# thnak/image_super_resolution

Measured on AMD Instinct MI355X. Metric: 4x SR megapixels/sec (HR output) + PSNR vs reference CPU path, higher is better.
Workload: dtype fp16; 1 GPU; ResNet(16, 0.2, scaleRate=4) RRDB inference, 128x128->512x512; global_batch=16, per_gpu_batch=16, lr_size=128, scale=4, parallelism=dp1 (independent tile shards), streams_per_gpu=1, hip_graph=True, trunk=persistent chain kernel, storage=fp16 activations and packed weights, fp32 accumulation

## Files before the change

### image_super_resolution_amd/csrc/capi.hip

```cpp
#include <stdarg.h>
#include <stdio.h>
#include <string.h>

#include "isr_common.h"

namespace isr {
int conv3x3_fwd_dispatch(const isr_conv_desc* d, hipStream_t s);
int conv3x3_fwd_variant(const isr_conv_desc* d, int variant, hipStream_t s);
int conv_stamps_set(void* p);
size_t trunk_state_words(int n, int ha, int wa);
int trunk_launch(const isr_chain_desc* c, hipStream_t s);
int trunk_stamps_set(void* p);
int trunk_knobs_set(const int* k);
int trunk_item_stamps_set(void* p);
size_t conv3x3_packed_bytes(int cout, int cin);
int conv3x3_pack(const float* w, void* out, int cout, int cin, hipStream_t s);
int conv3x3_pack_f16(const float* w, void* out, int cout, int cin, hipStream_t s);
size_t conv3x3_wino_packed_bytes(int cout, int cin);
int conv3x3_wino_pack(const float* w, void* out, int cout, int cin, hipStream_t s);
int conv3x3_wino_fwd_dispatch(const isr_conv_desc* d, hipStream_t s);
int head9x9_fwd_dispatch(const isr_head_desc* d, hipStream_t s);
int tail9x9_fwd_dispatch(const isr_tail_desc* d, hipStream_t s);
int tail9x9_fwd_variant(const isr_tail_desc* d, int variant, hipStream_t s);
size_t head9x9_packed_bytes(int cout);
// ... 32 lines not shown

static thread_local char g_err[512] = "";

static int fail(int code, const char* fmt, ...) __attribute__((format(printf, 2, 3)));
static int fail(int code, const char* fmt, ...) {
    va_list ap;
    va_start(ap, fmt);
    vsnprintf(g_err, sizeof(g_err), fmt, ap);
    va_end(ap);
    return code;
}

static int launched(int rc, const char* what) {
    if (rc != 0) {
        hipError_t e = hipGetLastError();
        return fail(ISR_ERR_LAUNCH, "%s: launch failed: %s", what, hipGetErrorString(e));
    }
    g_err[0] = 0;
    return ISR_OK;
}

static bool view_ok(const isr_view& v, int ha, int wa, int halo, int ch, const char* name, int align16) {
    if (!v.data) { fail(ISR_ERR_BAD_DESC, "%s: null data", name); return false; }
    if (v.pad < halo) { fail(ISR_ERR_BAD_DESC, "%s: pad %d < required halo %d", name, v.pad, halo); return false; }
    if (v.hp < ha + 2 * v.pad || v.wp < wa + 2 * v.pad) {
        fail(ISR_ERR_BAD_DESC, "%s: buffer %dx%d (pad %d) smaller than computed region %dx%d", name, v.hp, v.wp, v.pad, ha, wa);
        return false;
    }
    if (v.coff < 0 || v.coff + ch > v.cs) {
        fail(ISR_ERR_BAD_DESC, "%s: channels [%d,%d) exceed stride %d", name, v.coff, v.coff + ch, v.cs);
        return false;
    }
    if (align16 && ((v.cs % 16) || (v.coff % 16) || ((uintptr_t)v.data % 16))) {
        fail(ISR_ERR_BAD_DESC, "%s: channel count/offset must be multiples of 16 (channel-blocked layout) "
             "and data 16-byte aligned", name);
        return false;
    }
    return true;
}

extern "C" {

const char* isr_last_error(void) { return g_err; }

int isr_pack_conv3x3_batch(const isr_pack_item* items, int32_t n, isr_stream_t s) {
    if (!items || n <= 0 || n > 65535) return fail(ISR_ERR_BAD_DESC, "pack_conv3x3_batch: bad item table (n=%d)", n);
    return launched(isr::conv3x3_pack_batch(items, n, (hipStream_t)s), "pack_conv3x3_batch");
}

static int mt_ok(const isr_mt_tensor* ts, const isr_mt_chunk* cs, int32_t n, const char* what) {
    if (!ts || !cs) return fail(ISR_ERR_BAD_DESC, "%s: null tensor / chunk table", what);
    if (n <= 0 || n > (1 << 30)) return fail(ISR_ERR_BAD_DESC, "%s: bad chunk count %d", what, n);
    return ISR_OK;
}

int isr_mt_adam_guarded(const isr_mt_tensor* ts, const isr_mt_chunk* cs, int32_t n, const isr_adam_args* a,
                        const float* scale, const uint32_t* guard, isr_stream_t s) {
    if (int rc = mt_ok(ts, cs, n, "mt_adam")) return rc;
    if (!a) return fail(ISR_ERR_BAD_DESC, "mt_adam: null args");
    if (!(a->bc2_sqrt > 0.f) || !(a->beta1 >= 0.f && a->beta1 < 1.f) || !(a->beta2 >= 0.f && a->beta2 < 1.f))
        return fail(ISR_ERR_BAD_DESC, "mt_adam: bad betas / bias correction");
    return launched(isr::mt_adam_dispatch(ts, cs, n, a, scale, guard, (hipStream_t)s), "mt_adam");
}

int isr_mt_adam(const isr_mt_tensor* ts, const isr_mt_chunk* cs, int32_t n, const isr_adam_args* a,
                const float* scale, isr_stream_t s) {
    return isr_mt_adam_guarded(ts, cs, n, a, scale, nullptr, s);
}

int isr_mt_sumsq(const isr_mt_tensor* ts, const isr_mt_chunk* cs, int32_t n, float* partial, isr_stream_t s) {
    if (int rc = mt_ok(ts, cs, n, "mt_sumsq")) return rc;
    if (!partial) return fail(ISR_ERR_BAD_DESC, "mt_sumsq: null partial buffer");
    return launched(isr::mt_sumsq_dispatch(ts, cs, n, partial, (hipStream_t)s), "mt_sumsq");
}

int isr_clip_coef(const float* partial, int32_t n, float max_norm, float* out, isr_stream_t s) {
    if (!partial || !out || n <= 0) return fail(ISR_ERR_BAD_DESC, "clip_coef: bad arguments");
    return launched(isr::clip_coef_dispatch(partial, n, max_norm, out, (hipStream_t)s), "clip_coef");
}

int isr_mt_scale(const isr_mt_tensor* ts, const isr_mt_chunk* cs, int32_t n, const float* coef, isr_stream_t s) {
    if (int rc = mt_ok(ts, cs, n, "mt_scale")) return rc;
    if (!coef) return fail(ISR_ERR_BAD_DESC, "mt_scale: null coefficient");
    return launched(isr::mt_axpby_dispatch(ts, cs, n, 0, coef, 0.f, nullptr, (hipStream_t)s), "mt_scale");
}

int isr_mt_lerp_guarded(const isr_mt_tensor* ts, const isr_mt_chunk* cs, int32_t n, float d, const uint32_t* guard,
                        isr_stream_t s) {
    if (int rc = mt_ok(ts, cs, n, "mt_lerp")) return rc;
    return launched(isr::mt_axpby_dispatch(ts, cs, n, 1, nullptr, d, guard, (hipStream_t)s), "mt_lerp");
}

int isr_mt_lerp(const isr_mt_tensor* ts, const isr_mt_chunk* cs, int32_t n, float d, isr_stream_t s) {
    return isr_mt_lerp_guarded(ts, cs, n, d, nullptr, s);
}
int isr_version(void) { return 1; }

size_t isr_conv3x3_packed_bytes(int32_t cout, int32_t cin) { return isr::conv3x3_packed_bytes(cout, cin); }
size_t isr_head9x9_packed_bytes(int32_t cout, int32_t cin) { (void)cin; return isr::head9x9_packed_bytes(cout); }
size_t isr_tail9x9_packed_bytes(int32_t cout, int32_t cin) { (void)cout; (void)cin; return isr::tail9x9_packed_bytes(); }

int isr_pack_conv3x3(const float* w, void* packed, int32_t cout, int32_t cin, isr_stream_t s) {
    if (!w || !packed) return fail(ISR_ERR_BAD_DESC, "pack_conv3x3: null pointer");
    if (cin <= 0 || cin % 16) return fail(ISR_ERR_UNSUPPORTED, "pack_conv3x3: cin %d must be a positive multiple of 16", cin);
    if (cout <= 0 || cout % 32)
        return fail(ISR_ERR_UNSUPPORTED, "pack_conv3x3: cout %d must be a positive multiple of 32", cout);
    return launched(isr::conv3x3_pack(w, packed, cout, cin, (hipStream_t)s), "pack_conv3x3");
}

int isr_pack_conv3x3_dgrad(const float* w, void* packed, int32_t cout, int32_t cin, float scale, int32_t sub2,
                           isr_stream_t s) {
    if (!w || !packed) return fail(ISR_ERR_BAD_DESC, "pack_conv3x3_dgrad: null pointer");
    if (cin <= 0 || cin % 32 || cout <= 0 || cout % 32)
        return fail(ISR_ERR_UNSUPPORTED, "pack_conv3x3_dgrad: cin %d / cout %d must be multiples of 32", cin, cout);
    if (sub2 && cout % 128) return fail(ISR_ERR_UNSUPPORTED, "pack_conv3x3_dgrad: sub2 needs cout %% 128 == 0");
    return launched(isr::conv3x3_pack_dgrad(w, packed, cout, cin, scale, sub2, (hipStream_t)s), "pack_conv3x3_dgrad");
}

static int pack_head_any(const float* w, void* packed, int32_t cout, int32_t cin, isr_stream_t s, bool h) {
    if (!w || !packed) return fail(ISR_ERR_BAD_DESC, "pack_head9x9: null pointer");
    if (cout != 64 || cin < 1 || cin > 3) return fail(ISR_ERR_UNSUPPORTED, "pack_head9x9: need cout 64, cin <= 3 (got %d, %d)", cout, cin);
    return launched(isr::head9x9_pack(w, packed, cout, cin, (hipStream_t)s, h), "pack_head9x9");
}
int isr_pack_head9x9(const float* w, void* packed, int32_t cout, int32_t cin, isr_stream_t s) {
    return pack_head_any(w, packed, cout, cin, s, false);
}
int isr_pack_head9x9_f16(const float* w, void* packed, int32_t cout, int32_t cin, isr_stream_t s) {
    return pack_head_any(w, packed, cout, cin, s, true);
}

static int pack_tail_any(const float* w, void* packed, int32_t cout, int32_t cin, isr_stream_t s, bool h) {
    if (!w || !packed) return fail(ISR_ERR_BAD_DESC, "pack_tail9x9: null pointer");
    if (cout != 3 || cin != 64) return fail(ISR_ERR_UNSUPPORTED, "pack_tail9x9: need cout 3, cin 64 (got %d, %d)", cout, cin);
    return launched(isr::tail9x9_pack(w, packed, cout, cin, (hipStream_t)s, h), "pack_tail9x9");
}
int isr_pack_tail9x9(const float* w, void* packed, int32_t cout, int32_t cin, isr_stream_t s) {
    return pack_tail_any(w, packed, cout, cin, s, false);
}
int isr_pack_tail9x9_f16(const float* w, void* packed, int32_t cout, int32_t cin, isr_stream_t s) {
    return pack_tail_any(w, packed, cout, cin, s, true);
}

int isr_pack_conv3x3_f16(const float* w, void* packed, int32_t cout, int32_t cin, isr_stream_t s) {
    if (!w || !packed) return fail(ISR_ERR_BAD_DESC, "pack_conv3x3_f16: null pointer");
    if (cin <= 0 || cin % 16) return fail(ISR_ERR_UNSUPPORTED, "pack_conv3x3_f16: cin %d must be a positive multiple of 16", cin);
    if (cout <= 0 || cout % 32)
        return fail(ISR_ERR_UNSUPPORTED, "pack_conv3x3_f16: cout %d must be a positive multiple of 32", cout);
    return launched(isr::conv3x3_pack_f16(w, packed, cout, cin, (hipStream_t)s), "pack_conv3x3_f16");
}

static int conv3x3_validate(const isr_conv_desc* d) {
    if (!d) return fail(ISR_ERR_BAD_DESC, "conv3x3: null descriptor");
    if (d->n <= 0 || d->h <= 0 || d->w <= 0) return fail(ISR_ERR_BAD_DESC, "conv3x3: empty problem n=%d h=%d w=%d", d->n, d->h, d->w);
    if (d->ha % ISR_TILE_H || d->wa % ISR_TILE_W || d->ha < d->h || d->wa < d->w)
        return fail(ISR_ERR_BAD_DESC, "conv3x3: computed region %dx%d must cover %dx%d and be a multiple of %dx%d", d->ha, d->wa,
                    d->h, d->w, ISR_TILE_H, ISR_TILE_W);
    if (d->cin <= 0 || d->cin % 16) return fail(ISR_ERR_UNSUPPORTED, "conv3x3: cin %d must be a multiple of 16", d->cin);
    if (d->cout <= 0 || d->cout % 32)
        return fail(ISR_ERR_UNSUPPORTED, "conv3x3: cout %d must be a positive multiple of 32", d->cout);
    if (!d->wpack) return fail(ISR_ERR_BAD_DESC, "conv3x3: null weights");
    if (d->shuffle != 1 && d->shuffle != 2) return fail(ISR_ERR_UNSUPPORTED, "conv3x3: shuffle must be 1 or 2");
    if (d->taps < 0 || d->taps > 2) return fail(ISR_ERR_UNSUPPORTED, "conv3x3: taps must be 0, 1 or 2");
    if (d->taps && d->cout % 64) return fail(ISR_ERR_UNSUPPORTED, "conv3x3: a 2x2 tap window needs cout %% 64 == 0");
    if (d->x_sub2) {
        if (d->cin % 128) return fail(ISR_ERR_UNSUPPORTED, "conv3x3: x_sub2 needs cin %% 128 == 0 (got %d)", d->cin);
        if (d->shuffle != 1) return fail(ISR_ERR_UNSUPPORTED, "conv3x3: x_sub2 with a shuffled store");
        if (!view_ok(d->x, 2 * d->ha, 2 * d->wa, 2, d->cin / 4, "conv3x3.x", 1)) return ISR_ERR_BAD_DESC;
    } else if (!view_ok(d->x, d->ha, d->wa, 1, d->cin, "conv3x3.x", 1)) {
        return ISR_ERR_BAD_DESC;
    }
    if (d->m.data) {
        if (d->y2.data) return fail(ISR_ERR_UNSUPPORTED, "conv3x3: mask epilogue takes no second output");
        if (d->m_c0 < 0 || d->m_c0 % 32) return fail(ISR_ERR_BAD_DESC, "conv3x3: m_c0 %d must be a multiple of 32", d->m_c0);
        if (d->shuffle == 2) {
            if (d->m_c0) return fail(ISR_ERR_UNSUPPORTED, "conv3x3: a shuffled store masks all channels (m_c0 = 0)");
            if (!view_ok(d->m, 2 * d->ha, 2 * d->wa, 0, d->cout / 4, "conv3x3.m", 1)) return ISR_ERR_BAD_DESC;
        } else if (!view_ok(d->m, d->ha, d->wa, 0, d->cout, "conv3x3.m", 1)) {
            return ISR_ERR_BAD_DESC;
        }
    }
    if (d->r1_cn < 0 || d->r1_cn % 32) return fail(ISR_ERR_BAD_DESC, "conv3x3: r1_cn %d must be a multiple of 32", d->r1_cn);
    if (d->shuffle == 2) {
        if (d->cout % 64) return fail(ISR_ERR_UNSUPPORTED, "conv3x3: pixel shuffle needs cout %% 64 == 0");
        if (d->r1.data || d->r2.data || d->y2.data)
            return fail(ISR_ERR_UNSUPPORTED, "conv3x3: pixel shuffle store takes no residual / second output");
        if (!view_ok(d->y, 2 * d->ha, 2 * d->wa, 0, d->cout / 4, "conv3x3.y", 1)) return ISR_ERR_BAD_DESC;
    } else {
        if (!view_ok(d->y, d->ha, d->wa, 0, d->cout, "conv3x3.y", 1)) return ISR_ERR_BAD_DESC;
        if (d->y2.data && !view_ok(d->y2, d->ha, d->wa, 0, d->cout, "conv3x3.y2", 1)) return ISR_ERR_BAD_DESC;
        if (d->r1.data && !view_ok(d->r1, d->ha, d->wa, 0, d->cout, "conv3x3.r1", 1)) return ISR_ERR_BAD_DESC;
        if (d->r2.data && !view_ok(d->r2, d->ha, d->wa, 0, d->cout, "conv3x3.r2", 1)) return ISR_ERR_BAD_DESC;
    }
    if (d->bias && ((uintptr_t)d->bias % 16)) return fail(ISR_ERR_BAD_DESC, "conv3x3: bias must be 16-byte aligned");
    if (d->f16 != 0 && d->f16 != 1) return fail(ISR_ERR_BAD_DESC, "conv3x3: f16 must be 0 or 1");
    if (d->f16 && (d->m.data || d->x_sub2 || d->taps))
        return fail(ISR_ERR_UNSUPPORTED, "conv3x3: fp16 activations are forward-only (no mask, x_sub2 or tap window)");
    return ISR_OK;
}

int isr_conv3x3_fwd(const isr_conv_desc* d, isr_stream_t s) {
    int rc = conv3x3_validate(d);
    if (rc != ISR_OK) return rc;
    return launched(isr::conv3x3_fwd_dispatch(d, (hipStream_t)s), "conv3x3");
}

int isr_conv3x3_check(const isr_conv_desc* d) { return conv3x3_validate(d); }

size_t isr_conv3x3_wino_packed_bytes(int32_t cout, int32_t cin) {
    if (cout <= 0 || cin <= 0) return 0;
    return isr::conv3x3_wino_packed_bytes(cout, cin);
}

int isr_pack_conv3x3_wino_f16(const float* w, void* packed, int32_t cout, int32_t cin, isr_stream_t s) {
    if (!w || !packed) return fail(ISR_ERR_BAD_DESC, "pack_conv3x3_wino_f16: null pointer");
    if (cin <= 0 || cin % 16)
        return fail(ISR_ERR_UNSUPPORTED, "pack_conv3x3_wino_f16: cin %d must be a positive multiple of 16", cin);
    if (cout <= 0 || cout % 32)
        return fail(ISR_ERR_UNSUPPORTED, "pack_conv3x3_wino_f16: cout %d must be a positive multiple of 32", cout);
    return launched(isr::conv3x3_wino_pack(w, packed, cout, cin, (hipStream_t)s), "pack_conv3x3_wino_f16");
}

int isr_conv3x3_wino_fwd(const isr_conv_desc* d, isr_stream_t s) {
    if (!d) return fail(ISR_ERR_BAD_DESC, "conv3x3_wino: null descriptor");
    if (d->f16 != 1) return fail(ISR_ERR_UNSUPPORTED, "conv3x3_wino: f16 must be 1 (fp16 storage only, got %d)", d->f16);
    if (d->shuffle != 1) return fail(ISR_ERR_UNSUPPORTED, "conv3x3_wino: shuffle must be 1 (plain store, got %d)", d->shuffle);
    if (d->m.data) return fail(ISR_ERR_UNSUPPORTED, "conv3x3_wino: m (mask epilogue) is not supported");
    if (d->x_sub2) return fail(ISR_ERR_UNSUPPORTED, "conv3x3_wino: x_sub2 is not supported");
    if (d->taps) return fail(ISR_ERR_UNSUPPORTED, "conv3x3_wino: taps (tap window) is not supported");
    int rc = conv3x3_validate(d);
    if (rc != ISR_OK) return rc;
    return launched(isr::conv3x3_wino_fwd_dispatch(d, (hipStream_t)s), "conv3x3_wino");
}

size_t isr_conv_chain_state_words(int32_t n, int32_t ha, int32_t wa) {
    if (n <= 0 || ha <= 0 || wa <= 0 || ha % 16 || wa % 32) return 0;
    return isr::trunk_state_words(n, ha, wa);
}

#define ISR_REMOVED_FORM "is a removed A/B form (its measurements: DESIGN.md section 5)"

int isr_conv_chain_variant(const isr_chain_desc* c, int32_t variant, isr_stream_t s) {
    if (!c || !c->layers || !c->kinds || !c->state || c->nl <= 0 || c->nl > 1024)
        return fail(ISR_ERR_BAD_DESC, "conv chain: null layers / kinds / state or nl not in [1, 1024]");
    if (c->n <= 0 || c->ha <= 0 || c->wa <= 0 || c->ha % 16 || c->wa % 32)
        return fail(ISR_ERR_BAD_DESC, "conv chain: bad grid n=%d ha=%d wa=%d", c->n, c->ha, c->wa);
    if (c->f16 != 0 && c->f16 != 1) return fail(ISR_ERR_BAD_DESC, "conv chain: f16 must be 0 or 1");
    if (variant != 0) return fail(ISR_ERR_UNSUPPORTED, "conv chain: variant %d " ISR_REMOVED_FORM, variant);
    const int rc = isr::trunk_launch(c, (hipStream_t)s);
    if (rc == -4) return fail(ISR_ERR_LAUNCH, "conv chain: the occupancy query admits no workgroup per CU");
    if (rc == -2) return fail(ISR_ERR_UNSUPPORTED, "conv chain: unsupported grid or layer count");
    return launched(rc, "conv chain");
}

int isr_conv_chain(const isr_chain_desc* c, isr_stream_t s) { return isr_conv_chain_variant(c, 0, s); }

int isr_tuning_trunk_knobs(int32_t ablate, int32_t per_cu, int32_t k2, int32_t k3) {
    const int k[4] = {ablate, per_cu, k2, k3};
    const int rc = isr::trunk_knobs_set(k);
    if (rc == -2) return fail(ISR_ERR_UNSUPPORTED, "trunk knobs: library built without -DISR_TUNING");
    return rc == 0 ? ISR_OK : fail(ISR_ERR_LAUNCH, "trunk knobs: hipMemcpyToSymbol failed");
}

int isr_tuning_trunk_item_stamps(void* buf) {
    const int rc = isr::trunk_item_stamps_set(buf);
    if (rc == -2) return fail(ISR_ERR_UNSUPPORTED, "trunk item stamps: library built without -DISR_TUNING");
    return rc == 0 ? ISR_OK : fail(ISR_ERR_LAUNCH, "trunk item stamps: hipMemcpyToSymbol failed");
}

int isr_tuning_trunk_stamps(void* buf) {
    const int rc = isr::trunk_stamps_set(buf);
    if (rc == -2) return fail(ISR_ERR_UNSUPPORTED, "trunk stamps: library built without -DISR_TUNING");
    return rc == 0 ? ISR_OK : fail(ISR_ERR_LAUNCH, "trunk stamps: hipMemcpyToSymbol failed");
}

int isr_tuning_conv_stamps(void* buf) {
    const int rc = isr::conv_stamps_set(buf);
    if (rc == -2) return fail(ISR_ERR_UNSUPPORTED, "conv stamps: library built without -DISR_TUNING");
    return rc == 0 ? ISR_OK : fail(ISR_ERR_LAUNCH, "conv stamps: hipMemcpyToSymbol failed");
}

int isr_tuning_chain_knobs(int32_t, int32_t, int32_t, int32_t) {
    return fail(ISR_ERR_UNSUPPORTED, "chain knobs: the round-2 chain kernel that read them " ISR_REMOVED_FORM);
}

int isr_tuning_tail_stamps(void*) {
    return fail(ISR_ERR_UNSUPPORTED, "tail stamps: the 4-wave tail walk that wrote them " ISR_REMOVED_FORM);
}

int isr_conv3x3_fwd_variant(const isr_conv_desc* d, int32_t variant, isr_stream_t s) {
    int rc = conv3x3_validate(d);
    if (rc != ISR_OK) return rc;
    rc = isr::conv3x3_fwd_variant(d, variant, (hipStream_t)s);
    if (rc == -2) return fail(ISR_ERR_UNSUPPORTED, "conv3x3: variant %d not available for cout %d / cin %d", variant, d->cout, d->cin);
    return launched(rc, "conv3x3");
}

int isr_head9x9_fwd(const isr_head_desc* d, isr_stream_t s) {
    if (!d) return fail(ISR_ERR_BAD_DESC, "head9x9: null descriptor");
    if (d->n <= 0 || d->h <= 0 || d->w <= 0) return fail(ISR_ERR_BAD_DESC, "head9x9: empty problem");
    if (d->ha % ISR_TILE_H || d->wa % ISR_TILE_W || d->ha < d->h || d->wa < d->w)
        return fail(ISR_ERR_BAD_DESC, "head9x9: bad computed region %dx%d for %dx%d", d->ha, d->wa, d->h, d->w);
    if (d->cout != 64) return fail(ISR_ERR_UNSUPPORTED, "head9x9: cout must be 64");
    if (!d->x || !d->wpack) return fail(ISR_ERR_BAD_DESC, "head9x9: null input or weights");
    if (!view_ok(d->y, d->ha, d->wa, 0, 64, "head9x9.y", 1)) return ISR_ERR_BAD_DESC;
    if (d->y2.data && !view_ok(d->y2, d->ha, d->wa, 0, 64, "head9x9.y2", 1)) return ISR_ERR_BAD_DESC;
    if (d->m.data && !view_ok(d->m, d->ha, d->wa, 0, 64, "head9x9.m", 1)) return ISR_ERR_BAD_DESC;
    if (d->bias && ((uintptr_t)d->bias % 16)) return fail(ISR_ERR_BAD_DESC, "head9x9: bias must be 16-byte aligned");
    if (d->f16 != 0 && d->f16 != 1) return fail(ISR_ERR_BAD_DESC, "head9x9: f16 must be 0 or 1");
    if (d->f16 && d->m.data) return fail(ISR_ERR_UNSUPPORTED, "head9x9: fp16 activations are forward-only (no mask)");
// ... 380 lines not shown
```

### image_super_resolution_amd/csrc/conv3x3.hip

```cpp
#include <string.h>

#include "isr_common.h"

namespace isr {

#ifdef ISR_TUNING
__device__ unsigned long long* g_conv_stamps;
#endif
__device__ __forceinline__ void conv_stamp(int slot) {
#ifdef ISR_TUNING
    unsigned long long* p = g_conv_stamps;
    if (p != nullptr && threadIdx.x == 0) {
        unsigned long long t;
        asm volatile("s_memrealtime %0\n\ts_waitcnt lgkmcnt(0)" : "=s"(t)::"memory");
        p[(size_t)blockIdx.x * 8 + slot + threadIdx.x] = t;
        if (slot == 0) {
            const unsigned hw = __builtin_amdgcn_s_getreg((31 << 11) | (0 << 6) | 4);
            const unsigned xcc = __builtin_amdgcn_s_getreg((15 << 11) | (0 << 6) | 20);
            p[(size_t)blockIdx.x * 8 + 6 + threadIdx.x] = hw;
            p[(size_t)blockIdx.x * 8 + 7 + threadIdx.x] = xcc;
        }
    }
#else
    (void)slot;
// ... 440 lines not shown
                                    __builtin_amdgcn_sched_barrier(0);
                                    ++m;
                                }
                            }
                        }
                        if constexpr (FC >= 0 && C::FOLD && C::NF == 2 && C::KS == 1 && C::TN == 3) {
                            if (st == 1 && ia >= 1 && ia <= R) {
                                const bf16x8 a = fold_a(fidv, FC & 1);
                                acc[ia - 1][FC >> 1] = mfma32t<C::H>(a, fa[cur][ia], acc[ia - 1][FC >> 1]);
                                __builtin_amdgcn_sched_barrier(0);
                            }
                        }
                    }
                    continue;
                } else if constexpr (C::PIPE) {
                    if (st + 1 < NS) load_step(st + 1, cur ^ 1);
                    __builtin_amdgcn_sched_barrier(0);
                } else {
                    load_step(st, 0);
                }
    #pragma unroll
                for (int ia = 0; ia < NA; ++ia) {
    #pragma unroll
                    for (int dyi = 0; dyi < TN; ++dyi) {
                        const int r = ia - dyi;
                        if (r >= 0 && r < R) {
    #pragma unroll
                            for (int f = 0; f < NF; ++f) {
                                if constexpr (C::ABL & 1) {
                                    asm volatile("" ::"v"(fa[cur][ia]), "v"(fb[cur][dyi][f]));
                                } else {
                                    acc[r][f] = mfma32t<C::H>(fb[cur][dyi][f], fa[cur][ia], acc[r][f]);
                                }
                            }
                        }
                    }
                }
            }
#if ISR_CONV_PRIO
        __builtin_amdgcn_s_setprio(0);
#endif
    };
    int chunk0 = 0;
    if constexpr (C::FOLD && C::NF == 2 && C::KS == 1 && C::TN == 3) {
        if (fold && nchunks >= 4) {
            do_chunk(0, IC<0>{});
            do_chunk(1, IC<1>{});
            do_chunk(2, IC<2>{});
            do_chunk(3, IC<3>{});
            chunk0 = 4;
        }
    }
#pragma nounroll
    for (int chunk = chunk0; chunk < nchunks; ++chunk) do_chunk(chunk, IC<-1>{});
    asm volatile("s_waitcnt lgkmcnt(0)" ::: "memory");
    __builtin_amdgcn_s_barrier();
    conv_stamp(2);

    if constexpr (C::ABL & 4) {
        if (d.n < 0) {
            float s = 0.f;
#pragma unroll
            for (int r = 0; r < R; ++r)
#pragma unroll
                for (int f = 0; f < NF; ++f)
#pragma unroll
                    for (int g = 0; g < 16; ++g) s += acc[r][f][g];
            ((float*)d.y.data)[threadIdx.x] = s;
        }
        return;
    }
    const int mode = d.shuffle == 2 ? (d.m.data ? 24 : 8)
                     : fold ? (32 | (d.r2.data ? 2 : 0))
                            : ((d.r1.data ? 1 : 0) | (d.r2.data ? 2 : 0) | (d.y2.data ? 4 : 0) | (d.m.data ? 16 : 0));
    switch (mode) {
        case 32: epilogue<C, 32>(d, acc, img, ct, x0, y0, wave, lane); break;
        case 34: epilogue<C, 34>(d, acc, img, ct, x0, y0, wave, lane); break;
        case 0: epilogue<C, 0>(d, acc, img, ct, x0, y0, wave, lane); break;
        case 1: epilogue<C, 1>(d, acc, img, ct, x0, y0, wave, lane); break;
        case 2: epilogue<C, 2>(d, acc, img, ct, x0, y0, wave, lane); break;
        case 3: epilogue<C, 3>(d, acc, img, ct, x0, y0, wave, lane); break;
        case 4: epilogue<C, 4>(d, acc, img, ct, x0, y0, wave, lane); break;
        case 5: epilogue<C, 5>(d, acc, img, ct, x0, y0, wave, lane); break;
        case 6: epilogue<C, 6>(d, acc, img, ct, x0, y0, wave, lane); break;
        case 7: epilogue<C, 7>(d, acc, img, ct, x0, y0, wave, lane); break;
        case 8: epilogue<C, 8>(d, acc, img, ct, x0, y0, wave, lane); break;
        case 24: epilogue<C, 24>(d, acc, img, ct, x0, y0, wave, lane); break;
        case 16: epilogue<C, 16>(d, acc, img, ct, x0, y0, wave, lane); break;
        case 17: epilogue<C, 17>(d, acc, img, ct, x0, y0, wave, lane); break;
        case 18: epilogue<C, 18>(d, acc, img, ct, x0, y0, wave, lane); break;
        default: epilogue<C, 19>(d, acc, img, ct, x0, y0, wave, lane); break;
    }
#ifdef ISR_TUNING
    asm volatile("s_waitcnt vmcnt(0)" ::: "memory");
    conv_stamp(3);
#endif
}

template <class C, bool XS2>
__global__ __launch_bounds__(C::NT, C::OCC) void conv3x3_fwd_kernel(isr_conv_desc d) {
    conv_tile<C, XS2>(d, xcd_remap(blockIdx.x, gridDim.x));
}

template <class C, bool XS2>
static int launch3x3_k(const isr_conv_desc* d, hipStream_t s) {
    auto kern = conv3x3_fwd_kernel<C, XS2>;
    lds_limit((const void*)kern, C::LDS);
    const int blocks = (d->wa / C::TW) * (d->ha / C::TH) * d->n * (d->cout / C::CT);
    hipLaunchKernelGGL(kern, dim3(blocks), dim3(C::NT), C::LDS, s, *d);
    return hipGetLastError() == hipSuccess ? 0 : -1;
}

template <class C, bool FULL = false>
static int launch3x3(const isr_conv_desc* d, hipStream_t s) {
    if (d->cout % C::CT || d->cin % C::KC || d->ha % C::TH) return -2;
    if (C::CIN && d->cin != C::CIN) return -2;
    if constexpr (FULL) {
        if (d->x_sub2) return launch3x3_k<C, true>(d, s);
    } else {
        if (d->x_sub2) return -2;
    }
    return launch3x3_k<C, false>(d, s);
}

using V_G0 = C3<4, 4, 1, 16, 2, 0, 0, 2>;
using V_G1 = C3<4, 8, 1, 16, 3>;
using V_G2 = C3<2, 4, 1, 32, 2>;
using V_G3 = C3<2, 4, 1, 16, 2, 0, 0, 2>;
using V_W0 = C3<4, 4, 2, 16, 2, 0, 0, 2>;
using V_W1 = C3<4, 8, 2, 16, 2>;
using V_W2 = C3<2, 4, 2, 32, 2>;
using V_W3 = C3<2, 4, 2, 16, 2, 0, 0, 2>;
using V_F0 = C3<4, 4, 2, 16, 2, 192, 0, 2>;
using V_F0F = C3<4, 4, 2, 16, 2, 192, 0, 2, 4, 0, 0, 0, 1>;
using V_G0H = C3<4, 4, 1, 16, 2, 0, 0, 2, 4, 0, 0, 0, 0, 1>;
using V_W0H = C3<4, 4, 2, 16, 2, 0, 0, 2, 4, 0, 0, 0, 0, 1>;
using V_F0H = C3<4, 4, 2, 16, 2, 192, 0, 2, 4, 0, 0, 0, 0, 1>;
using V_F0FH = C3<4, 4, 2, 16, 2, 192, 0, 2, 4, 0, 0, 0, 1, 1>;

static bool fold_host(const isr_conv_desc* d) {
    if (!d->r1.data || d->r1.data != d->x.data || d->r1.coff != d->x.coff || d->r1_cn != 0) return false;
    if (d->cout != 64 || d->slope != 1.f || d->y2.data || d->m.data || d->shuffle != 1 || d->x_sub2 || d->taps)
        return false;
    const float inv = 1.f / d->s1;
    uint32_t bits;
    memcpy(&bits, &inv, 4);
    if (d->f16) {
        const int ex = (int)((bits >> 23) & 0xff) - 127;
        return (bits & 0x1fffu) == 0 && ex >= -14 && ex <= 15;
    }
    return (bits & 0xffffu) == 0;
}

int conv3x3_fwd_variant(const isr_conv_desc* d, int variant, hipStream_t s) {
    if (d->f16) {
        if (variant != 0 || d->x_sub2 || d->taps || d->m.data) return -2;
        if (d->cout % 64) return launch3x3<V_G0H>(d, s);
        return d->cin == 192 ? (fold_host(d) ? launch3x3<V_F0FH>(d, s) : launch3x3<V_F0H>(d, s)) : launch3x3<V_W0H>(d, s);
    }
    if (d->cout % 64) {
        switch (variant) {
            case 0: return launch3x3<V_G0, true>(d, s);
#ifdef ISR_TUNING
            case 1: return launch3x3<V_G1>(d, s);
            case 2: return launch3x3<V_G2>(d, s);
            case 3: return launch3x3<V_G3>(d, s);
            case 8: return launch3x3<C3<4, 4, 1, 16, 2, 0, 0, 2, 4, 1>>(d, s);
            case 9: return launch3x3<C3<4, 8, 1, 16, 2, 0, 0, 2>>(d, s);
            case 4: return launch3x3<C3<4, 4, 1, 16, 2, 0, 1>>(d, s);
            case 5: return launch3x3<C3<4, 4, 1, 16, 2, 0, 2>>(d, s);
            case 6: return launch3x3<C3<4, 4, 1, 16, 2, 0, 4>>(d, s);
            case 7: return launch3x3<C3<4, 4, 1, 16, 2, 0, 3>>(d, s);
#endif
        }
        return -2;
    }
    switch (variant) {
        case 0: return d->cin == 192 ? (fold_host(d) ? launch3x3<V_F0F>(d, s) : launch3x3<V_F0, true>(d, s))
                                     : launch3x3<V_W0, true>(d, s);
#ifdef ISR_TUNING
        case 1: return launch3x3<V_W1>(d, s);
        case 2: return launch3x3<V_W2>(d, s);
        case 3: return launch3x3<V_W3>(d, s);
        case 8: return d->cin == 192 ? launch3x3<C3<4, 4, 2, 16, 2, 192, 0, 2, 4, 1>>(d, s)
                                     : launch3x3<C3<4, 4, 2, 16, 2, 0, 0, 2, 4, 1>>(d, s);
        case 9: return d->cin == 192 ? launch3x3<C3<4, 8, 2, 16, 2, 192, 0, 2>>(d, s)
                                     : launch3x3<C3<4, 8, 2, 16, 2, 0, 0, 2>>(d, s);
        case 10: return launch3x3<C3<4, 4, 2, 16, 2, 0, 8, 2>>(d, s);
        case 11: return launch3x3<C3<4, 8, 2, 16, 2, 0, 8, 2>>(d, s);
        case 4: return launch3x3<C3<4, 4, 2, 16, 2, 0, 1>>(d, s);
        case 5: return launch3x3<C3<4, 4, 2, 16, 2, 0, 2>>(d, s);
        case 6: return launch3x3<C3<4, 4, 2, 16, 2, 0, 4>>(d, s);
        case 7: return launch3x3<C3<4, 4, 2, 16, 2, 0, 3>>(d, s);
#endif
    }
    return -2;
}

#ifdef ISR_TUNING
int conv_stamps_set(void* p) { return hipMemcpyToSymbol(HIP_SYMBOL(g_conv_stamps), &p, sizeof(p)) == hipSuccess ? 0 : -1; }
#else
int conv_stamps_set(void*) { return -2; }
#endif

int conv3x3_fwd_dispatch(const isr_conv_desc* d, hipStream_t s) {
    if (d->f16) return conv3x3_fwd_variant(d, 0, s);
    if (d->taps == 1) return d->cout % 64 ? -2 : launch3x3<C3<4, 4, 2, 16, 2, 0, 0, 0, 4, 1, 1>, true>(d, s);
    if (d->taps == 2) return d->cout % 64 ? -2 : launch3x3<C3<4, 4, 2, 16, 2, 0, 0, 0, 4, 1, 2>, true>(d, s);
    return conv3x3_fwd_variant(d, 0, s);
}

template <class OT = __bf16>
__device__ __forceinline__ void pack3x3_range(const float* __restrict__ w, OT* __restrict__ out, int pcout,
                                              int pcin, int transposed, int sub2, float scale, size_t first,
                                              size_t stride, int src_n0 = 0, int src_cin = 0) {
    const int wrow = src_cin > 0 ? src_cin : pcout;
    const size_t total = (size_t)pcout * pcin * 9;
    for (size_t idx = first; idx < total; idx += stride) {
        size_t rem = idx;
        const int e = rem % 8; rem /= 8;
        const int hpos = rem % 2; rem /= 2;
        const int n = rem % pcout; rem /= pcout;
        const int tap = rem % 9; rem /= 9;
        const int c16 = (int)rem;
        const int h = hpos ^ ((n >> 3) & 1);
        const int ci = c16 * 16 + h * 8 + e;
        float v;
        if (!transposed) {
            v = w[((size_t)n * pcin + ci) * 9 + tap];
        } else {
            const int cs4 = pcin >> 2;
            const int co = sub2 ? (ci % cs4) * 4 + ci / cs4 : ci;
            v = w[((size_t)co * wrow + src_n0 + n) * 9 + (8 - tap)];
        }
        out[idx] = (OT)(v * scale);
    }
}

template <class OT>
__global__ void pack3x3_kernel(const float* __restrict__ w, OT* __restrict__ out, int pcout, int pcin,
                               int transposed, int sub2, float scale) {
    pack3x3_range<OT>(w, out, pcout, pcin, transposed, sub2, scale, blockIdx.x * (size_t)blockDim.x + threadIdx.x,
                      (size_t)gridDim.x * blockDim.x);
}

__global__ void pack3x3_batch_kernel(const isr_pack_item* __restrict__ items) {
    const isr_pack_item it = items[blockIdx.y];
    const int pcout = it.dgrad ? it.cin : it.cout, pcin = it.dgrad ? it.cout : it.cin;
    pack3x3_range(it.w, (__bf16*)it.out, pcout, pcin, it.dgrad, it.sub2, it.dgrad ? it.scale : 1.f,
                  blockIdx.x * (size_t)blockDim.x + threadIdx.x, (size_t)gridDim.x * blockDim.x,
                  it.dgrad ? it.src_n0 : 0, it.dgrad ? it.src_cin : 0);
}

int conv3x3_pack_batch(const isr_pack_item* items, int n, hipStream_t s) {
    hipLaunchKernelGGL(pack3x3_batch_kernel, dim3(96, n), dim3(256), 0, s, items);
    return hipGetLastError() == hipSuccess ? 0 : -1;
}

size_t conv3x3_packed_bytes(int cout, int cin) { return (size_t)cout * cin * 9 * 2; }

static int pack_launch(const float* w, void* out, int pcout, int pcin, int transposed, int sub2, float scale,
                       hipStream_t s) {
    const size_t total = conv3x3_packed_bytes(pcout, pcin) / 2;
    const int blocks = (int)((total + 255) / 256 < 4096 ? (total + 255) / 256 : 4096);
    hipLaunchKernelGGL(pack3x3_kernel<__bf16>, dim3(blocks), dim3(256), 0, s, w, (__bf16*)out, pcout, pcin, transposed,
                       sub2, scale);
    return hipGetLastError() == hipSuccess ? 0 : -1;
}

int conv3x3_pack(const float* w, void* out, int cout, int cin, hipStream_t s) {
    return pack_launch(w, out, cout, cin, 0, 0, 1.f, s);
}

int conv3x3_pack_f16(const float* w, void* out, int cout, int cin, hipStream_t s) {
    const size_t total = conv3x3_packed_bytes(cout, cin) / 2;
    const int blocks = (int)((total + 255) / 256 < 4096 ? (total + 255) / 256 : 4096);
    hipLaunchKernelGGL(pack3x3_kernel<_Float16>, dim3(blocks), dim3(256), 0, s, w, (_Float16*)out, cout, cin, 0, 0,
                       1.f);
    return hipGetLastError() == hipSuccess ? 0 : -1;
}

int conv3x3_pack_dgrad(const float* w, void* out, int cout, int cin, float scale, int sub2, hipStream_t s) {
    return pack_launch(w, out, cin, cout, 1, sub2, scale, s);
}

}
```

Measured before the change: 671.2 MPix/s.

## Add persistent streaming kernel for pixel-shuffle upscaler conv3x3

Adds a persistent kernel for the shuffle-2 upsampling 3x3 convolutions, used by default when the descriptor qualifies. Each workgroup walks a contiguous range of tiles and output-channel blocks. It double-buffers halo and weight chunks into LDS through buffer-load-to-LDS and prefetches the next item's first chunk during the last chunk of the current one. The epilogue fuses LeakyReLU with a DPP lane permutation so pixel-shuffled stores are wider and contiguous. This is meant to cut per-tile launch and prologue cost and overlap loads with MFMA, at the cost of a large, complex kernel and a relaxed tile-height validation for this path.

```diff
diff --git a/image_super_resolution_amd/csrc/capi.hip b/image_super_resolution_amd/csrc/capi.hip
--- a/image_super_resolution_amd/csrc/capi.hip
+++ b/image_super_resolution_amd/csrc/capi.hip
@@ -208,9 +208,10 @@
 static int conv3x3_validate(const isr_conv_desc* d) {
     if (!d) return fail(ISR_ERR_BAD_DESC, "conv3x3: null descriptor");
     if (d->n <= 0 || d->h <= 0 || d->w <= 0) return fail(ISR_ERR_BAD_DESC, "conv3x3: empty problem n=%d h=%d w=%d", d->n, d->h, d->w);
-    if (d->ha % ISR_TILE_H || d->wa % ISR_TILE_W || d->ha < d->h || d->wa < d->w)
+    const int tile_h = d->shuffle == 2 && d->cout % 64 == 0 && !d->x_sub2 && !d->taps ? 16 : ISR_TILE_H;
+    if (d->ha % tile_h || d->wa % ISR_TILE_W || d->ha < d->h || d->wa < d->w)
         return fail(ISR_ERR_BAD_DESC, "conv3x3: computed region %dx%d must cover %dx%d and be a multiple of %dx%d", d->ha, d->wa,
-                    d->h, d->w, ISR_TILE_H, ISR_TILE_W);
+                    d->h, d->w, tile_h, ISR_TILE_W);
     if (d->cin <= 0 || d->cin % 16) return fail(ISR_ERR_UNSUPPORTED, "conv3x3: cin %d must be a multiple of 16", d->cin);
     if (d->cout <= 0 || d->cout % 32)
         return fail(ISR_ERR_UNSUPPORTED, "conv3x3: cout %d must be a positive multiple of 32", d->cout);
diff --git a/image_super_resolution_amd/csrc/conv3x3.hip b/image_super_resolution_amd/csrc/conv3x3.hip
--- a/image_super_resolution_amd/csrc/conv3x3.hip
+++ b/image_super_resolution_amd/csrc/conv3x3.hip
@@ -616,7 +616,20 @@
     return (bits & 0xffffu) == 0;
 }
 
+bool scaler_stream_ok(const isr_conv_desc* d);
+int scaler_stream_launch(const isr_conv_desc* d, int cap, hipStream_t s, int probe = 0);
+
+static int conv3x3_per_tile(const isr_conv_desc* d, int variant, hipStream_t s);
+
 int conv3x3_fwd_variant(const isr_conv_desc* d, int variant, hipStream_t s) {
+    if (variant == 13) return scaler_stream_launch(d, 3, s);
+    if (variant >= 14 && variant <= 19) return scaler_stream_launch(d, 0, s, variant - 13);
+    if (variant == 12) return conv3x3_per_tile(d, 0, s);
+    if (variant == 0 && scaler_stream_ok(d)) return scaler_stream_launch(d, 0, s);
+    return conv3x3_per_tile(d, variant, s);
+}
+
+static int conv3x3_per_tile(const isr_conv_desc* d, int variant, hipStream_t s) {
     if (d->f16) {
         if (variant != 0 || d->x_sub2 || d->taps || d->m.data) return -2;
         if (d->cout % 64) return launch3x3<V_G0H>(d, s);
diff --git a/image_super_resolution_amd/csrc/scaler_stream.hip b/image_super_resolution_amd/csrc/scaler_stream.hip
--- /dev/null
+++ b/image_super_resolution_amd/csrc/scaler_stream.hip
@@ -0,0 +1,351 @@
+#include "trunk_common.h"
+
+namespace isr {
+
+struct SS {
+    static constexpr int WM = 4, R = 4, NST = 2;
+    static constexpr int NT = 64 * WM;
+    static constexpr int TH = tk::TH;
+    static constexpr int HQ = tk::HQ;
+    static constexpr int HP = tk::HP;
+    static constexpr int WP = tk::WPF;
+    static_assert(R * WM == TH, "the waves cover the tile rows");
+    static_assert(HP % WM == 0, "every wave stages the same number of halo pieces");
+    static constexpr int HPW = HP / WM;
+    static constexpr int WPW = (WP + WM - 1) / WM;
+    static constexpr int SLOT = (HP + WP) * 1024;
+    static constexpr int BIAS_OFF = NST * SLOT;
+    static constexpr int LDS = BIAS_OFF + 4 * 256;
+    static constexpr int BPC = 2;
+    static_assert(LDS <= 81920, "two workgroups per CU (tests/test_scaler_stream_resources.py reads this bound)");
+    static constexpr int WPS = BPC * WM / 4;
+    static constexpr int STORES = R * 4;
+};
+
+struct ScalerArgs {
+    const char* x;
+    char* y;
+    const char* w;
+    const float* bias;
+    uint32_t xplane, yplane, wbytes;
+    int32_t x_cs16, x_p0, x_wp, x_pad;
+    int32_t y_cs16, y_p0, y_wp, y_pad;
+    int32_t h, wv, nbx, nby, ntiles, nch, nct, cout;
+    float slope;
+};
+
+struct SItem {
+    const char* xb;
+    uint32_t h0;
+    int ct, img, x0, y0;
+};
+
+constexpr int SS_PROD = 8;
+template <bool H, int FORM = SS_PROD>
+__global__ __launch_bounds__(SS::NT, SS::WPS) void scaler_stream_kernel(ScalerArgs a) {
+    extern __shared__ __attribute__((aligned(16))) char smem[];
+    constexpr int R = SS::R, NF = 2, CT = 64, TN = 3, NA = R + 2;
+    const int wave = wave_id(), lane = threadIdx.x & 63, l31 = lane & 31, hh = lane >> 5;
+    const int G = (int)gridDim.x, b = xcd_remap((int)blockIdx.x, G);
+    const int t0 = (int)((unsigned long long)b * (unsigned)a.ntiles / (unsigned)G);
+    const int t1 = (int)((unsigned long long)(b + 1) * (unsigned)a.ntiles / (unsigned)G);
+    const int nct = a.nct, nch = a.nch;
+    const int nitems = (t1 - t0) * nct;
+    if (nitems <= 0) return;
+
+    auto item_of = [&](int i) {
+        const int ti = i / nct;
+        const int t = t0 + ti;
+        const int bx = t % a.nbx, tmp = t / a.nbx, by = tmp % a.nby;
+        SItem it;
+        it.ct = i - ti * nct;
+        it.img = tmp / a.nby;
+        it.x0 = bx * tk::TW;
+        it.y0 = by * SS::TH;
+        it.xb = a.x + (size_t)((uint32_t)it.img * a.x_cs16 + a.x_p0) * a.xplane;
+        it.h0 = (uint32_t)(((it.y0 - 1 + a.x_pad) * a.x_wp + (it.x0 - 1 + a.x_pad)) * 32);
+        return it;
+    };
+
+    uint32_t hoff[SS::HPW];
+#pragma unroll
+    for (int k = 0; k < SS::HPW; ++k) hoff[k] = halo_piece_off<SS::HQ>(wave + SS::WM * k, lane, a.x_wp);
+
+    auto stage = [&](const SItem& it, int chunk, int slot, bool with_bias, int bslot, bool first = false) {
+        if constexpr ((FORM & 2) != 0) {
+            if (!first && a.ntiles >= 0) return;
+        }
+        char* dst = smem + slot * SS::SLOT;
+        const auto rx = rsrc_n(it.xb + (size_t)chunk * a.xplane, a.xplane);
+#pragma unroll
+        for (int k = 0; k < SS::HPW; ++k) {
+            const int j = wave + SS::WM * k;
+            __builtin_amdgcn_raw_ptr_buffer_load_lds(rx, ISR_LDS_PTR(dst + j * 1024), 16, hoff[k], it.h0, 0, 0);
+        }
+        const auto rw = rsrc_n(a.w, a.wbytes);
+        const uint32_t wo = (uint32_t)((chunk * 9 * a.cout + it.ct * CT) * 32);
+#pragma unroll
+        for (int k = 0; k < SS::WPW; ++k) {
+            const int j = wave + SS::WM * k;
+            if (SS::WM * k + SS::WM <= SS::WP || j < SS::WP)
+                __builtin_amdgcn_raw_ptr_buffer_load_lds(rw, ISR_LDS_PTR(dst + (SS::HP + j) * 1024), 16, lane * 16,
+                                                         wo + (uint32_t)((j >> 1) * a.cout * 32 + (j & 1) * 1024), 0, 0);
+        }
+        if (with_bias && wave == 0)
+            __builtin_amdgcn_raw_ptr_buffer_load_lds(rsrc_n(a.bias + it.ct * CT, 256u),
+                                                     ISR_LDS_PTR(smem + SS::BIAS_OFF + bslot * 256), 4, lane * 4, 0, 0, 0);
+    };
+
+    const uint32_t a_w = (uint32_t)(SS::HP * 1024 + (2 * l31 + (hh ^ ((l31 >> 3) & 1))) * 16);
+    uint32_t a_h[3];
+#pragma unroll
+    for (int dx = 0; dx < 3; ++dx)
+        a_h[dx] = (uint32_t)((wave * R * tk::HC + l31 + dx) * 32 + 16 * (hh ^ (((l31 + dx) >> 3) & 1)));
+
+    f32x16 acc[R][NF];
+    SItem cur = item_of(0), nxt = cur;
+    int slot = 0;
+    uint32_t pend = 0;
+    stage(cur, 0, 0, true, 0, true);
+
+    for (int i = 0; i < nitems; ++i) {
+        const int bslot = i & 3;
+        auto do_chunk = [&](const int ch, auto first_tag) {
+            constexpr bool FIRST = decltype(first_tag)::value != 0;
+            if constexpr (FIRST) wait_vm_coarse(pend);
+            else asm volatile("s_waitcnt vmcnt(0)" ::: "memory");
+            raw_barrier();
+            if constexpr (FIRST) {
+                const float* bs = reinterpret_cast<const float*>(smem + SS::BIAS_OFF + bslot * 256);
+#pragma unroll
+                for (int f = 0; f < NF; ++f) {
+                    f32x16 b0;
+#pragma unroll
+                    for (int j = 0; j < 4; ++j) {
+                        const f32x4 q = *reinterpret_cast<const f32x4*>(bs + f * 32 + 8 * j + 4 * hh);
+#pragma unroll
+                        for (int e = 0; e < 4; ++e) b0[4 * j + e] = q[e];
+                    }
+#pragma unroll
+                    for (int r = 0; r < R; ++r) acc[r][f] = b0;
+                }
+            }
+            const char* sb = smem + slot * SS::SLOT;
+            bf16x8 fb[2][TN][NF], fa[2][NA];
+            auto read_one = [&](int dx, int idx, int set) {
+                if (idx < TN * NF) {
+                    const int dyi = idx / NF, f = idx % NF;
+                    fb[set][dyi][f] = lds_read16(sb + a_w + ((dyi * 3 + dx) * CT * 2 + f * 64) * 16);
+                } else {
+                    const int ia = idx - TN * NF;
+                    fa[set][ia] = lds_read16(sb + a_h[dx] + ia * tk::HC * 32);
+                }
+            };
+            auto read_fb = [&](int dx, int dyi, int set) {
+#pragma unroll
+                for (int f = 0; f < NF; ++f) read_one(dx, dyi * NF + f, set);
+            };
+            read_fb(0, 0, 0);
+#pragma unroll
+            for (int ia = 0; ia < R; ++ia) read_one(0, TN * NF + ia, 0);
+            read_fb(0, 1, 0);
+            read_one(0, TN * NF + R, 0);
+            read_fb(0, 2, 0);
+            read_one(0, TN * NF + R + 1, 0);
+            __builtin_amdgcn_sched_barrier(0);
+
+            if constexpr (FIRST) {
+                stage(cur, 1, slot ^ 1, false, 0);
+            } else {
+                const bool last = ch == nch - 1;
+                if (!last) {
+                    stage(cur, ch + 1, slot ^ 1, false, 0);
+                } else if (i + 1 < nitems) {
+                    nxt = item_of(i + 1);
+                    stage(nxt, 0, slot ^ 1, true, (bslot + 1) & 3);
+                }
+            }
+            __builtin_amdgcn_sched_barrier(0);
+            __builtin_amdgcn_s_setprio(1);
+#pragma unroll
+            for (int stp = 0; stp < 3; ++stp) {
+                const int cs = stp & 1;
+#pragma unroll
+                for (int dyi = 0; dyi < TN; ++dyi) {
+#pragma unroll
+                    for (int r = 0; r < R; ++r) {
+#pragma unroll
+                        for (int f = 0; f < NF; ++f) acc[r][f] = mfma32t<H>(fb[cs][dyi][f], fa[cs][r + dyi], acc[r][f]);
+                        if (stp + 1 < 3 && (dyi == 2 || r == 0)) read_one(stp + 1, TN * NF + r + dyi, cs ^ 1);
+                        __builtin_amdgcn_sched_barrier(0);
+                    }
+                    if (stp + 1 < 3) {
+                        read_fb(stp + 1, dyi, cs ^ 1);
+                        __builtin_amdgcn_sched_barrier(0);
+                    }
+                }
+            }
+            __builtin_amdgcn_s_setprio(0);
+            slot ^= 1;
+        };
+        do_chunk(0, TIC<1>{});
+#pragma nounroll
+        for (int ch = 1; ch < nch; ++ch) do_chunk(ch, TIC<0>{});
+
+        {
+            asm volatile("; scaler stream epilogue");
+            typedef __attribute__((ext_vector_type(2))) float f32x2;
+            typedef __attribute__((ext_vector_type(4))) unsigned u32x4;
+            const float slope = a.slope;
+            const auto yr = rsrc_n(a.y + (size_t)((uint32_t)cur.img * a.y_cs16 + a.y_p0 + cur.ct) * a.yplane, a.yplane);
+            const int xx = cur.x0 + l31;
+#pragma unroll
+            for (int r = 0; r < R; ++r) {
+                const int yy = cur.y0 + wave * R + r;
+                const bool valid = yy < a.h && xx < a.wv;
+                const uint32_t off = (uint32_t)(((2 * yy + hh + a.y_pad) * a.y_wp + 2 * xx + a.y_pad) * 32);
+                float v[NF][16];
+#pragma unroll
+                for (int f = 0; f < NF; ++f) {
+                    const f32x16& c = acc[r][f];
+#pragma unroll
+                    for (int g = 0; g < 16; g += 2) {
+                        const f32x2 p = f32x2{c[g], c[g + 1]} * slope;
+                        v[f][g] = c[g] >= 0.f ? c[g] : p[0];
+                        v[f][g + 1] = c[g + 1] >= 0.f ? c[g + 1] : p[1];
+                    }
+#pragma unroll
+                    for (int j = 0; j < 4; ++j) {
+                        swap_halves(v[f][4 * j], v[f][4 * j + 2]);
+                        swap_halves(v[f][4 * j + 1], v[f][4 * j + 3]);
+                    }
+                }
+                u32x4 z[4];
+#pragma unroll
+                for (int sj = 0; sj < 2; ++sj)
+#pragma unroll
+                    for (int f = 0; f < NF; ++f) {
+                        float u[8];
+#pragma unroll
+                        for (int j = 0; j < 4; ++j) {
+                            u[2 * j] = v[f][4 * j + sj];
+                            u[2 * j + 1] = v[f][4 * j + 2 + sj];
+                        }
+                        u32x4 t = __builtin_bit_cast(u32x4, pack8_pairs<H>(u));
+#pragma unroll
+                        for (int k = 0; k < 4; ++k) t[k] = valid ? t[k] : 0u;
+                        z[2 * sj + f] = t;
+                    }
+                uint32_t so = off;
+                if constexpr ((FORM & 8) != 0) {
+                    const bool b0 = (lane & 1) != 0, b1 = (lane & 2) != 0;
+                    auto x1 = [](uint32_t q) { return (uint32_t)__builtin_amdgcn_mov_dpp((int)q, 0xB1, 0xf, 0xf, true); };
+                    auto x2 = [](uint32_t q) { return (uint32_t)__builtin_amdgcn_mov_dpp((int)q, 0x4E, 0xf, 0xf, true); };
+#pragma unroll
+                    for (int k = 0; k < 4; ++k) {
+#pragma unroll
+                        for (int p = 0; p < 4; p += 2) {
+                            const uint32_t lo = z[p][k], hi = z[p + 1][k];
+                            const uint32_t plo = x1(lo), phi = x1(hi);
+                            z[p][k] = b0 ? phi : lo;
+                            z[p + 1][k] = b0 ? hi : plo;
+                        }
+#pragma unroll
+                        for (int p = 0; p < 2; ++p) {
+                            const uint32_t lo = z[p][k], hi = z[p + 2][k];
+                            const uint32_t plo = x2(lo), phi = x2(hi);
+                            z[p][k] = b1 ? phi : lo;
+                            z[p + 2][k] = b1 ? hi : plo;
+                        }
+                    }
+                    so = off - (uint32_t)((lane & 3) * 48);
+                }
+                constexpr int PSTEP = (FORM & 8) ? 64 : 16;
+                constexpr int SAUX = (FORM & 16) ? 2 : 0;
+#pragma unroll
+                for (int q = 0; q < 4; ++q) {
+                    bool go = true;
+                    if constexpr ((FORM & 1) != 0) go = a.ntiles < 0;
+                    if constexpr ((FORM & 4) != 0) go = z[q][0] == 0x7fc12345u;
+                    if (go) __builtin_amdgcn_raw_buffer_store_b128(z[q], yr, so + (uint32_t)(q * PSTEP), 0, SAUX);
+                }
+            }
+        }
+        pend = SS::STORES;
+        cur = nxt;
+    }
+}
+
+bool scaler_stream_ok(const isr_conv_desc* d) {
+    if (d->shuffle != 2 || d->m.data || d->taps || d->x_sub2 || d->y2.data || d->r1.data || d->r2.data) return false;
+    if (d->cout % 64 || d->cin % 16 || d->cin < 32 || d->ha % SS::TH || d->wa % tk::TW) return false;
+    if (!d->bias || !d->wpack || d->y.data == d->x.data) return false;
+    if (d->x.coff % 16 || d->x.cs % 16 || d->y.coff % 16 || d->y.cs % 16 || d->x.pad < 1 || d->y.pad < 0) return false;
+    if ((size_t)d->x.hp * d->x.wp * 32 >= 0x7fffffffull || (size_t)d->y.hp * d->y.wp * 32 >= 0x7fffffffull) return false;
+    if ((size_t)d->cout * d->cin * 18 >= 0x7fffffffull) return false;
+    const long long ntiles = (long long)d->n * (d->ha / SS::TH) * (d->wa / tk::TW);
+    return ntiles > 0 && ntiles <= (1 << 24);
+}
+
+template <bool H, int FORM = SS_PROD>
+static int scaler_stream_launch_k(const isr_conv_desc* d, int cap, hipStream_t s) {
+    static thread_local int cached_dev = -1, cached_per_cu = 0, cached_cus = 0;
+    int dev = 0;
+    if (hipGetDevice(&dev) != hipSuccess) return -1;
+    const void* kern = (const void*)scaler_stream_kernel<H, FORM>;
+    if (dev != cached_dev) {
+        (void)hipFuncSetAttribute(kern, hipFuncAttributeMaxDynamicSharedMemorySize, SS::LDS);
+        int per_cu = 0;
+        if (hipOccupancyMaxActiveBlocksPerMultiprocessor(&per_cu, kern, SS::NT, SS::LDS) != hipSuccess) return -1;
+        int cus = 0;
+        if (hipDeviceGetAttribute(&cus, hipDeviceAttributeMultiprocessorCount, dev) != hipSuccess || cus <= 0) return -1;
+        cached_dev = dev;
+        cached_per_cu = per_cu < 1 ? 1 : (per_cu < SS::BPC ? per_cu : SS::BPC);
+        cached_cus = cus;
+    }
+    ScalerArgs a;
+    a.x = (const char*)d->x.data;
+    a.y = (char*)d->y.data;
+    a.w = (const char*)d->wpack;
+    a.bias = d->bias;
+    a.xplane = (uint32_t)((size_t)d->x.hp * d->x.wp * 32);
+    a.yplane = (uint32_t)((size_t)d->y.hp * d->y.wp * 32);
+    a.wbytes = (uint32_t)((size_t)d->cout * d->cin * 18);
+    a.x_cs16 = d->x.cs / 16;
+    a.x_p0 = d->x.coff / 16;
+    a.x_wp = d->x.wp;
+    a.x_pad = d->x.pad;
+    a.y_cs16 = d->y.cs / 16;
+    a.y_p0 = d->y.coff / 16;
+    a.y_wp = d->y.wp;
+    a.y_pad = d->y.pad;
+    a.h = d->h;
+    a.wv = d->w;
+    a.nbx = d->wa / tk::TW;
+    a.nby = d->ha / SS::TH;
+    a.ntiles = d->n * a.nbx * a.nby;
+    a.nch = d->cin / 16;
+    a.nct = d->cout / 64;
+    a.cout = d->cout;
+    a.slope = d->slope;
+    long long grid = (long long)cached_per_cu * cached_cus;
+    if (cap > 0 && cap < grid) grid = cap;
+    if (a.ntiles < grid) grid = a.ntiles;
+    hipLaunchKernelGGL((scaler_stream_kernel<H, FORM>), dim3((unsigned)grid), dim3(SS::NT), SS::LDS, s, a);
+    return hipGetLastError() == hipSuccess ? 0 : -1;
+}
+
+int scaler_stream_launch(const isr_conv_desc* d, int cap, hipStream_t s, int probe) {
+    if (!scaler_stream_ok(d)) return -2;
+#ifdef ISR_TUNING
+#define ISR_SS_FORM(p, k) \
+    if (probe == p) return d->f16 ? scaler_stream_launch_k<true, k>(d, cap, s) : scaler_stream_launch_k<false, k>(d, cap, s);
+    ISR_SS_FORM(1, SS_PROD | 1) ISR_SS_FORM(2, SS_PROD | 2) ISR_SS_FORM(3, SS_PROD | 3) ISR_SS_FORM(4, SS_PROD | 4)
+    ISR_SS_FORM(5, 0) ISR_SS_FORM(6, SS_PROD | 16)
+#undef ISR_SS_FORM
+#endif
+    if (probe != 0) return -2;
+    return d->f16 ? scaler_stream_launch_k<true>(d, cap, s) : scaler_stream_launch_k<false>(d, cap, s);
+}
+
+}
```

Measured after the change: 677.7 MPix/s (median of 6 runs). No clear change (+1.0%).
